# wafgo/rt-depth-map

Hardware: AMD Instinct MI355X
Metric: stereo-pairs/sec, 1280x720 d=64 9x9 SAD (higher is better)
Workload: dtype u8

## Files before the change

rt-depth-map_amd/csrc/k_search_ring.hip:

```cpp
#include "rtdm_select.h"
#include "rtdm_border.h"
#include "rtdm_border2.h"
#include "rtdm_search.h"

#include <cmath>
#include <cstdlib>
#include <type_traits>
#include <utility>

namespace rtdm {

struct RingGeom {
    int x0, nx;
    int rs;
    uint32_t lastmask;
    int tiles, strips;
    unsigned nitems;
    unsigned chunk;
    uint32_t rdelta;
    int rebase;
    unsigned nborder;
    int bgx, bgy;
    int b2;
};

__host__ __device__ constexpr int ring_rpg(int D, int LPP) { return D >= 96 ? 4 : LPP; }

template <int D, int WS, int LPP = 2>
struct RingCfg {
    static constexpr int RPG = ring_rpg(D, LPP);
    static constexpr bool SPLIT = LPP != 2 || D >= 48 || (D == 32 && (WS == 9 || WS == 5));
    static constexpr bool B64 = SPLIT && D == 64;
    using Rec = SelRecord<D, B64>;
    static constexpr int NP = (WS + 3) / 4;
    static constexpr int W1 = WS + 1;
    static constexpr int PPW = 64 / LPP;
    static constexpr bool PAIR = D == 64 && WS == 9 && LPP == 4;
    static constexpr int LPG = PAIR ? 2 * LPP : LPP;
    static constexpr int GPW = 64 / LPG;
    static constexpr int DL = D / LPG;
    static constexpr int NGL = DL / 4;
    static constexpr int NRL = DL / 2;
    static constexpr int NL = PAIR ? NP + 1 : NP;
    static constexpr int NW = NGL + NL - 1;
    static constexpr int LWD = GPW + NP;
    static constexpr int RWD = GPW + D / 4 + NP;
    static constexpr int ITEMS = (LWD + RWD + 63) / 64;
    static constexpr int SLOT = ITEMS * 64;
    static constexpr int TRIP = (W1 % RPG == 0) ? W1 : (2 * W1 % RPG == 0) ? 2 * W1 : 4 * W1;
    static_assert(W1 % 2 == 0 && TRIP % RPG == 0 && TRIP % W1 == 0, "block sizes are odd");
    static constexpr bool STATIC_SLOTS = ITEMS == 1 && TRIP % 4 == 0;
    static constexpr int NSLOT = STATIC_SLOTS ? 4 : 3;
    static constexpr int TEXD = (PAIR ? (TRIP + RPG) : (W1 + RPG)) * PPW / 2;
    static constexpr int STG = (NSLOT * SLOT + TEXD + 3) & ~3;
    static constexpr int PREC = D / 2 + D / 16;
    static constexpr int PREC_PAIR = LPG * PREC;
    __host__ __device__ static constexpr int pair_rec(int p, int o) { return p * PREC_PAIR + o * PREC + 2 * (p & 1) + 8 * (p >> 1); }
    static constexpr int REC_DWORDS = PAIR ? pair_rec(GPW - 1, LPG - 1) + PREC + 2 : PPW * RPG * Rec::DWORDS;
    static constexpr int WAVE_LDS = STG + REC_DWORDS;
    static constexpr int RING_REGS = W1 * NRL * (PAIR ? 2 : 1);
    static constexpr int W3_LIMIT = 112;
    static constexpr int WAVES = PAIR ? 3 : LPP >= 8 ? 2 : LPP == 4 ? (RING_REGS <= 80 ? 4 : (RING_REGS <= 96 && NRL <= 8) ? 3 : 2) : (RING_REGS <= 72 && NRL <= 8) ? 4 : RING_REGS <= W3_LIMIT ? 3 : 2;
    static constexpr int TILE = 4 * PPW;
    static constexpr bool FUSE_BORDER = WAVES < 4 && !PAIR;
    static constexpr bool FUSE_BORDER2 = D <= 192;
    static constexpr bool ROW_PTRS = !(LPP == 2 && RING_REGS > 88 && WAVES == 3);
};

template <int D, int WS, int LPP, bool BORDER>
struct RingBounds {
    using C = RingCfg<D, WS, LPP>;
    static constexpr int WAVES = BORDER && C::WAVES > 1 && !C::PAIR ? C::WAVES - 1 : C::WAVES;
};

template <int D, int WS, int LPP = 2>
struct RingState {
    uint64_t P[RingCfg<D, WS, LPP>::W1][RingCfg<D, WS, LPP>::NGL];
    uint64_t P2[RingCfg<D, WS, LPP>::PAIR ? RingCfg<D, WS, LPP>::W1 : 1][RingCfg<D, WS, LPP>::NGL];
};

template <int D, int WS, int LPP = 2>
struct RowRegs { uint64_t win[RingCfg<D, WS, LPP>::NW]; uint32_t l[RingCfg<D, WS, LPP>::NL]; };

typedef __attribute__((address_space(3))) const uint32_t* lds_cptr;
__device__ __forceinline__ uint32_t lds_addr(const uint32_t* q) { return (uint32_t)(uintptr_t)(lds_cptr)q; }
__device__ __forceinline__ lds_cptr lds_at(uint32_t a) { return (lds_cptr)(uintptr_t)a; }

template <int D, int WS, int LPP, typename PTR>
__device__ __forceinline__ void ring_load_row(PTR lp, PTR rp, PTR rpo, RowRegs<D, WS, LPP>& rw)
{
    using C = RingCfg<D, WS, LPP>;
#pragma unroll
    for (int k = 0; k < C::NL; ++k) rw.l[k] = lp[k];
#pragma unroll
    for (int j = 0; j < C::NW; ++j) {
        const PTR wp = (j & 1) ? rpo + (j - 1) : rp + j;
        rw.win[j] = (uint64_t)wp[0] | ((uint64_t)wp[1] << 32);
    }
}

template <int D, int WS, int LPP, int K, int NRLc>
__device__ __forceinline__ void ring_step(RingState<D, WS, LPP>& st, const RowRegs<D, WS, LPP>& rw, uint32_t lastmask, uint32_t capb,
                                          uint32_t& tnew, uint32_t (&S)[NRLc])
{
    using C = RingCfg<D, WS, LPP>;
    auto& P = st.P;
    constexpr int NP = C::NP, NGL = C::NGL, W1 = C::W1;
    constexpr int KP = (K + W1 - 1) % W1, KO = (K + 1) % W1;
    uint32_t l[NP];
#pragma unroll
    for (int k = 0; k < NP; ++k) l[k] = rw.l[k];
    l[NP - 1] &= lastmask;
#pragma unroll
    for (int k = 0; k < NP - 1; ++k) tnew = __builtin_amdgcn_sad_u8(l[k], capb, tnew);
    tnew = __builtin_amdgcn_msad_u8(capb, l[NP - 1], tnew);
#pragma unroll
    for (int j = 0; j < C::NW; ++j) {
#pragma unroll
        for (int k = 0; k < NP; ++k) {
            const int gi = j - k;
            if (gi >= 0 && gi < NGL) {
                const uint64_t acc = k == 0 ? P[KP][gi] : P[K][gi];
                if (k == NP - 1) P[K][gi] = __builtin_amdgcn_mqsad_pk_u16_u8(rw.win[j], l[k], acc);
                else             P[K][gi] = __builtin_amdgcn_qsad_pk_u16_u8(rw.win[j], l[k], acc);
            }
        }
    }
#pragma unroll
    for (int gi = 0; gi < NGL; ++gi) {
        S[2 * gi] = (uint32_t)P[K][gi] - (uint32_t)P[KO][gi];
        S[2 * gi + 1] = (uint32_t)(P[K][gi] >> 32) - (uint32_t)(P[KO][gi] >> 32);
    }
}

__device__ __forceinline__ uint64_t ring_add_halves(uint64_t a, uint64_t b)
{
    typedef uint32_t u2 __attribute__((ext_vector_type(2)));
    return __builtin_bit_cast(uint64_t, __builtin_bit_cast(u2, a) + __builtin_bit_cast(u2, b));
}

template <int D, int WS, int LPP, int K, int NRLc>
__device__ __forceinline__ void ring_step_pair(RingState<D, WS, LPP>& st, const RowRegs<D, WS, LPP>& rw, uint32_t (&S)[NRLc], uint32_t (&S2)[NRLc])
{
    using C = RingCfg<D, WS, LPP>;
    static_assert(C::PAIR && WS % 4 == 1, "the two windows share whole dwords only for w = 1 (mod 4)");
    constexpr int NP = C::NP, NGL = C::NGL, W1 = C::W1;
    constexpr int KP = (K + W1 - 1) % W1, KO = (K + 1) % W1;
    const uint32_t lf = rw.l[0] & 0xff000000u, ll = rw.l[NP] & 0x000000ffu;
    uint64_t sh[NGL], e1[NGL], e2[NGL];
#pragma unroll
    for (int j = 0; j < C::NW; ++j) {
#pragma unroll
        for (int k = 0; k <= NP; ++k) {
            const int gi = j - k;
            if (gi >= 0 && gi < NGL) {
                if (k == 0)       e1[gi] = __builtin_amdgcn_mqsad_pk_u16_u8(rw.win[j], lf, st.P[KP][gi]);
                else if (k == NP) e2[gi] = __builtin_amdgcn_mqsad_pk_u16_u8(rw.win[j], ll, st.P2[KP][gi]);
                else              sh[gi] = __builtin_amdgcn_qsad_pk_u16_u8(rw.win[j], rw.l[k], k == 1 ? (uint64_t)0 : sh[gi]);
            }
        }
    }
#pragma unroll
    for (int gi = 0; gi < NGL; ++gi) {
        st.P[K][gi] = ring_add_halves(e1[gi], sh[gi]);
        st.P2[K][gi] = ring_add_halves(e2[gi], sh[gi]);
        S[2 * gi] = (uint32_t)st.P[K][gi] - (uint32_t)st.P[KO][gi];
        S[2 * gi + 1] = (uint32_t)(st.P[K][gi] >> 32) - (uint32_t)(st.P[KO][gi] >> 32);
        S2[2 * gi] = (uint32_t)st.P2[K][gi] - (uint32_t)st.P2[KO][gi];
        S2[2 * gi + 1] = (uint32_t)(st.P2[K][gi] >> 32) - (uint32_t)(st.P2[KO][gi] >> 32);
    }
}

template <int N>
__device__ __forceinline__ void pin(uint32_t (&v)[N])
{
#pragma unroll
    for (int i = 0; i < N; ++i) asm volatile("" : "+v"(v[i]));
}

template <typename T>
__device__ __forceinline__ __attribute__((address_space(3))) T* lds_as(uint32_t a) { return (__attribute__((address_space(3))) T*)(uintptr_t)a; }

template <typename C>
struct RingTexture {
    static constexpr int TRIP = C::TRIP, RPG = C::RPG, WS = C::W1 - 1;
    static_assert(RPG == 4 && TRIP % RPG == 0 && TRIP >= WS + RPG && (WS - 1) % RPG == 0, "one straddling group, at U = w - 1");
    static constexpr int RING_BYTES = C::PPW * TRIP * 2;
    uint32_t a_row, a_edge;
    uint32_t a_term, a_col;
    uint32_t a_ring, a_wrap;
    uint32_t w_lo, w_hi;
    uint32_t carry;

    __device__ __forceinline__ void init(uint32_t stg_addr, uint32_t tex_addr, int p, int h)
    {
        const int k = h >> 1, j = h & 1, colw = 2 * p + j;
        a_row = stg_addr + (uint32_t)(k * C::SLOT + p + 1) * 4;
        a_edge = stg_addr + (uint32_t)(k * C::SLOT + p) * 4 + (j ? 12u : 3u);
        a_col = tex_addr + RING_BYTES + (uint32_t)colw * (RPG * 2);
        a_term = a_col + 2 * k;
        a_ring = tex_addr + (uint32_t)(colw * TRIP + k) * 2;
        a_wrap = tex_addr + (uint32_t)(colw * TRIP + (k + TRIP - 1) % TRIP) * 2;
        w_lo = k >= 1 ? 0x00010001u : 0x00000001u;
        w_hi = k >= 3 ? 0x00010001u : k == 2 ? 0x00000001u : 0u;
        carry = 0;
        asm volatile("" : "+v"(a_row), "+v"(a_edge), "+v"(a_term), "+v"(a_col), "+v"(a_ring), "+v"(a_wrap), "+v"(w_lo), "+v"(w_hi));
    }
    template <int U>
    __device__ __forceinline__ uint32_t back() const
    {
        constexpr int lo = U - WS;
        if constexpr (lo < 0 && lo + RPG - 1 >= 0) {
            static_assert(lo == -1, "a_wrap is the address for U = w - 1");
            return *lds_as<const uint16_t>(a_wrap);
        } else {
            constexpr int idx = (lo + TRIP) % TRIP;
            static_assert(idx + RPG - 1 < TRIP, "no wrap inside the group");
            return *lds_as<const uint16_t>(a_ring + idx * 2);
        }
    }
    __device__ __forceinline__ void term(uint32_t capb) const
    {
        const uint32_t l1 = *lds_as<const uint32_t>(a_row), l2 = *lds_as<const uint32_t>(a_row + 4);
        const uint32_t e = *lds_as<const uint8_t>(a_edge);
        uint32_t t = __builtin_amdgcn_sad_u8(l1, capb, 0u);
        t = __builtin_amdgcn_sad_u8(l2, capb, t);
        t = __builtin_amdgcn_msad_u8(capb, e, t);
        *lds_as<uint16_t>(a_term) = (uint16_t)t;
    }
    template <int U>
    __device__ __forceinline__ uint32_t prefix()
    {
        const uint64_t q = *lds_as<const uint64_t>(a_col);
        const sel_us2 lo = __builtin_bit_cast(sel_us2, (uint32_t)q), hi = __builtin_bit_cast(sel_us2, (uint32_t)(q >> 32));
        const sel_us2 ones = __builtin_bit_cast(sel_us2, 0x00010001u);
        uint32_t own = __builtin_amdgcn_udot2(lo, __builtin_bit_cast(sel_us2, w_lo), carry, false);
        own = __builtin_amdgcn_udot2(hi, __builtin_bit_cast(sel_us2, w_hi), own, false);
        carry = __builtin_amdgcn_udot2(lo, ones, carry, false);
        carry = __builtin_amdgcn_udot2(hi, ones, carry, false);
        *lds_as<uint16_t>(a_ring + U * 2) = (uint16_t)own;
        return own;
    }
};

template <typename F, int... U>
__device__ __forceinline__ void ring_for_groups(std::integer_sequence<int, U...>, F&& f)
{ (void)(f(std::integral_constant<int, U>{}) && ...); }
template <typename F, int... R>
__device__ __forceinline__ void ring_for_rows(std::integer_sequence<int, R...>, F&& f)
{ (f(std::integral_constant<int, R>{}), ...); }

template <int D, int WS, int LPP, bool FUSE>
__global__ __launch_bounds__(256, (RingBounds<D, WS, LPP, FUSE>::WAVES)) void k_search_ring(Plane8 Lp, Plane8 Rp, Plane16W disp, uint16_t* cost, BMGeom g, RingGeom rg,
                                                                                   BorderGeom bg, Border2Geom b2g)
{
    using C = RingCfg<D, WS, LPP>;
    constexpr int NGL = C::NGL, NRL = C::NRL, W1 = C::W1, LWD = C::LWD, SLOT = C::SLOT, ITEMS = C::ITEMS, PPW = C::PPW, RPG = C::RPG;
    constexpr int GPW = C::GPW;
    constexpr bool SPLIT = C::SPLIT, PAIR = C::PAIR;
    static_assert(!PAIR || (SPLIT && C::STATIC_SLOTS && C::LPG == 2 * RPG), "the paired layout: one owner lane per (column, row) of a group");
    constexpr int RECD = C::Rec::DWORDS;
    extern __shared__ __attribute__((aligned(16))) uint32_t lds[];

    unsigned fi = blockIdx.x;
    if constexpr (FUSE) {
        if (fi < rg.nborder) {
            const unsigned per = (unsigned)(rg.bgx * rg.bgy), fr = fi / per, id = fi - fr * per;
            if (C::FUSE_BORDER2 && rg.b2) {
                const int wave = __builtin_amdgcn_readfirstlane((int)(threadIdx.x >> 6));
                border2_body<D, C::NP>(Lp, Rp, disp, cost, g, b2g, (int)(id % rg.bgx) * 4 + wave, (int)(id / rg.bgx), (int)fr);
            } else if constexpr (C::FUSE_BORDER) {
                border_body<(D + 63) / 64>((unsigned char*)lds, Lp, Rp, disp, cost, g, bg, (int)(id % rg.bgx), (int)(id / rg.bgx), (int)fr);
            }
            return;
        }
        fi -= rg.nborder;
    }
    if (rg.chunk) fi = (fi & 7u) * rg.chunk + (fi >> 3);
    if (fi >= rg.nitems) return;
    const int b_tile = (int)(fi % rg.tiles), b_strip = (int)((fi / rg.tiles) % rg.strips), f = (int)(fi / (rg.tiles * rg.strips));

    const int tid = threadIdx.x, lane = tid & 63;
    const int phi = __builtin_amdgcn_readfirstlane(tid >> 6);
    const int p = lane & (GPW - 1), h = lane / GPW;
    const int x_tile = rg.x0 + b_tile * C::TILE;
    const int xw = PAIR ? x_tile + (phi >> 1) * (C::TILE / 2) + 2 * (phi & 1) : x_tile + phi;
    const int hrow = PAIR ? h >> 1 : h;
    const int x = xw + 4 * p + (PAIR ? h & 1 : 0);
    const bool active = x < rg.x0 + rg.nx;
    const int ys0 = g.vy0 + b_strip * rg.rs;
    const int ys1 = min(ys0 + rg.rs, g.vy1);
    if (ys0 >= ys1) return;
    const int r = g.r;
    const uint8_t* Lb = Lp.base + (size_t)f * Lp.frame;
    constexpr int PAIR_SHIFT = PAIR ? 3 : 0;
    const int Lbase = g.lofs + xw - r;
    const int Rbase = g.rofs + xw - r;
    const uint32_t capb = (uint32_t)(g.cap + PREFILTER_BIAS) * 0x01010101u;

    uint32_t* stg = lds + phi * C::WAVE_LDS;
    unsigned short* ptr = (unsigned short*)(stg + C::NSLOT * SLOT);
    unsigned short* ptw = ptr + W1 * PPW;
    const bool owner = PAIR || RPG == LPP || h < RPG;
    const unsigned short* ptw_own = ptw + (owner ? hrow : 0) * PPW + p;
    struct None {};
    [[maybe_unused]] std::conditional_t<PAIR, RingTexture<C>, None> tex;
    static_assert(!PAIR || ((C::NSLOT * SLOT) % 2 == 0 && C::WAVE_LDS % 2 == 0), "the row terms of a column are read as 8 bytes");
    uint32_t* scr = stg + C::STG + (PAIR ? C::pair_rec(p, h) : (owner ? lane : 0) * RECD);
    uint32_t* const rec0 = stg + C::STG + (PAIR ? C::pair_rec(p, 0) : p * RECD);
    uint32_t* scr_w = rec0 + h * NRL;
    using GSel = GroupSelectRec<D, C::LPG, C::B64>;
    unsigned short* scr_m = (unsigned short*)(rec0 + D / 2) + h * (NRL / 4);
    if constexpr (SPLIT) GSel::init(scr);

    const int row0 = ys0 - r;
    const int Hm1 = g.H - 1;
    const uint8_t* rowp = Lb + (size_t)row0 * Lp.pitch - PAIR_SHIFT;
    uint32_t loff[ITEMS];
#pragma unroll
    for (int it = 0; it < ITEMS; ++it) {
        const int idx = lane + it * 64;
        const bool isr = idx >= LWD;
        const int m = isr ? (PAIR ? min(idx - LWD, C::RWD - 1) : idx - LWD) : idx;
        loff[it] = (uint32_t)((isr ? Rbase : Lbase) + 4 * m) + (isr ? rg.rdelta : 0u);
    }
    int next_row = row0;
    uint32_t pre[2][ITEMS];
    auto issue = [&](auto Sc) {
        constexpr int SET = decltype(Sc)::value;
#pragma unroll
        for (int it = 0; it < ITEMS; ++it) {
            asm volatile("" : "+v"(loff[it]));
            pre[SET][it] = *(const uint32_t*)(rowp + loff[it]);
        }
        rowp += next_row < Hm1 ? Lp.pitch : 0;
        ++next_row;
    };
    auto commit = [&](auto Sc, auto slot) {
        constexpr int SET = decltype(Sc)::value;
#pragma unroll
        for (int it = 0; it < ITEMS; ++it) stg[slot * SLOT + lane + it * 64] = pre[SET][it];
        __builtin_amdgcn_wave_barrier();
    };
    using Set0 = std::integral_constant<int, 0>;
    using Set1 = std::integral_constant<int, 1>;

    RingState<D, WS, LPP> st;
#pragma unroll
    for (int k = 0; k < W1; ++k)
#pragma unroll
        for (int i = 0; i < NGL; ++i) {
            st.P[k][i] = 0;
            if constexpr (PAIR) st.P2[k][i] = 0;
        }
    if constexpr (PAIR) {
        constexpr int RINGD = RingTexture<C>::RING_BYTES / 4;
#pragma unroll
        for (int i = 0; i < (RINGD + 63) / 64; ++i)
            if (i * 64 + 63 < RINGD || lane + i * 64 < RINGD) stg[C::NSLOT * SLOT + lane + i * 64] = 0;
        tex.init(lds_addr(stg), lds_addr(stg + C::NSLOT * SLOT), p, h);
    } else {
#pragma unroll
        for (int k = 0; k < W1; ++k) ptr[k * PPW + p] = 0;
    }
    uint32_t pt = 0;

    const int nsteps = (ys1 - ys0) + WS - 1;
    const int nstepsg = (nsteps + RPG - 1) / RPG * RPG;
    issue(Set0{}); issue(Set1{});
    commit(Set0{}, 0); commit(Set1{}, 1);
    issue(Set0{});

    char* const db = (char*)(disp.base + (size_t)f * disp.frame_e);
    char* const cb = (char*)(cost + (size_t)f * g.H * g.Ws);
    const int col = g.lofs + x;
    constexpr int TF = (WS - 1) / RPG * RPG;
    uint32_t dofs = (uint32_t)(((long long)(ys0 + TF + hrow - (WS - 1)) * (long long)disp.pitch_e + col) * 2);
    uint32_t cofs = (uint32_t)(((long long)(ys0 + TF + hrow - (WS - 1)) * (long long)g.Ws + col) * 2);
    const uint32_t dstep = (uint32_t)(disp.pitch_e * 2 * RPG), cstep = (uint32_t)(g.Ws * 2 * RPG);
    const bool masked_col = g.mask_cols && (col < g.vx0 || col >= g.vx1);

    uint32_t S[RPG][NRL];
    int sl_cur = 0;
    uint32_t la_cur = lds_addr(stg + p), ra_cur = lds_addr(stg + LWD + p + h * NGL), ro_cur = ra_cur + 4;
    if constexpr (C::STATIC_SLOTS) asm volatile("" : "+v"(la_cur), "+v"(ra_cur), "+v"(ro_cur));
    const auto lds_row = [&](auto SLc, RowRegs<D, WS, LPP>& rw) {
        if constexpr (C::STATIC_SLOTS) {
            constexpr uint32_t off = (uint32_t)(decltype(SLc)::value * SLOT * 4);
            ring_load_row<D, WS, LPP>(lds_at(la_cur + off), lds_at(ra_cur + off), lds_at(ro_cur + off), rw);
        } else if constexpr (C::ROW_PTRS) {
            asm volatile("" : "+v"(la_cur), "+v"(ra_cur), "+v"(ro_cur));
            ring_load_row<D, WS, LPP>(lds_at(la_cur), lds_at(ra_cur), lds_at(ro_cur), rw);
            const uint32_t adv = (uint32_t)((sl_cur == 2 ? -2 * SLOT : SLOT) * 4);
            la_cur += adv; ra_cur += adv; ro_cur += adv;
        } else {
            int li = sl_cur * SLOT + p, ri = sl_cur * SLOT + LWD + p + h * NGL, one = 1;
            asm volatile("" : "+v"(li), "+v"(ri), "+v"(one));
            ring_load_row<D, WS, LPP, const uint32_t*>(stg + li, stg + ri, stg + ri + one, rw);
        }
    };
    [[maybe_unused]] uint32_t tback = 0, tpre = 0;
    auto step = [&](auto Kc, auto SLc, auto Rc, auto Uc, const RowRegs<D, WS, LPP>& rw, uint32_t (&Sr)[NRL], uint32_t (&Sr2)[NRL]) {
        constexpr int K = decltype(Kc)::value;
        using SetIn = std::integral_constant<int, (K + 1) & 1>;
        using SetOut = std::integral_constant<int, K & 1>;
        issue(SetIn{});
        uint32_t tnew = 0;
        constexpr int KO = (K + 1) % W1;
        if constexpr (PAIR) {
            constexpr int R = decltype(Rc)::value, U = decltype(Uc)::value;
            if constexpr (R == 2) { tback = tex.template back<U>(); tex.term(capb); }
            if constexpr (R == 3) tpre = tex.template prefix<U>();
            ring_step_pair<D, WS, LPP, K>(st, rw, Sr, Sr2);
            pin(Sr2);
        } else {
            ring_step<D, WS, LPP, K>(st, rw, rg.lastmask, capb, tnew, Sr);
            pt += tnew;
            const uint32_t told = ptr[KO * PPW + p];
            ptr[K * PPW + p] = (unsigned short)pt;
            ptw[decltype(Rc)::value * PPW + p] = (unsigned short)(pt - told);
        }
        pin(Sr);
        if constexpr (C::STATIC_SLOTS) {
            commit(SetOut{}, std::integral_constant<int, (decltype(SLc)::value + 2) % 4>{});
        } else {
            const int sl_new = sl_cur == 0 ? 2 : sl_cur - 1;
            sl_cur = sl_cur == 2 ? 0 : sl_cur + 1;
            commit(SetOut{}, sl_new);
        }
    };

    int trips_since_rebase = 0;
    for (int t0 = 0; t0 < nstepsg; t0 += C::TRIP) {
        if (rg.rebase && ++trips_since_rebase > rg.rebase) {
            trips_since_rebase = 1;
#pragma unroll
            for (int i = 0; i < NGL; ++i) {
                const uint32_t blo = (uint32_t)st.P[1][i], bhi = (uint32_t)(st.P[1][i] >> 32);
#pragma unroll
                for (int k = 1; k < W1; ++k) {
                    const uint32_t lo = (uint32_t)st.P[k][i] - blo, hi = (uint32_t)(st.P[k][i] >> 32) - bhi;
                    st.P[k][i] = (uint64_t)lo | ((uint64_t)hi << 32);
                }
                if constexpr (PAIR) {
                    const uint32_t blo2 = (uint32_t)st.P2[1][i], bhi2 = (uint32_t)(st.P2[1][i] >> 32);
#pragma unroll
                    for (int k = 1; k < W1; ++k) {
                        const uint32_t lo = (uint32_t)st.P2[k][i] - blo2, hi = (uint32_t)(st.P2[k][i] >> 32) - bhi2;
                        st.P2[k][i] = (uint64_t)lo | ((uint64_t)hi << 32);
                    }
                }
            }
        }
        ring_for_groups(std::make_integer_sequence<int, C::TRIP / RPG>{}, [&](auto Uc) -> bool {
            constexpr int U = RPG * decltype(Uc)::value;
            const int t = t0 + U;
            if (t >= nstepsg) return false;
            GSel gsel;
            ring_for_rows(std::make_integer_sequence<int, RPG>{}, [&](auto Rc) {
                constexpr int R = decltype(Rc)::value;
                RowRegs<D, WS, LPP> rw;
                using SL = std::integral_constant<int, (U + R) % 4>;
                lds_row(SL{}, rw);
                uint32_t S2[NRL] = {};
                step(std::integral_constant<int, (U + R) % W1>{}, SL{}, Rc, std::integral_constant<int, U>{}, rw, S[R], S2);
                if constexpr (PAIR) {
                    gsel.template row<R>(S[R], scr_w + 2 * R * C::PREC, scr_m + 2 * R * (C::PREC * 2));
                    gsel.template row<R>(S2, scr_w + (2 * R + 1) * C::PREC, scr_m + (2 * R + 1) * (C::PREC * 2));
                } else if constexpr (SPLIT) gsel.template row<R>(S[R], scr_w + R * (PPW * RECD), scr_m + R * (PPW * RECD * 2));
            });
            if (t + RPG - 1 < WS - 1) return true;
            const int y = ys0 + (t - (WS - 1)) + hrow;
            const bool row_ok = owner && y >= ys0 && y < ys1;
            const uint32_t dof = dofs, cof = cofs;
            dofs += dstep; cofs += cstep;
            int tsum;
            if constexpr (PAIR) tsum = (int)((tpre - tback) & 0xffffu);
            else tsum = *ptw_own;
            const bool dead = !active | !row_ok | masked_col | (tsum < g.tex);
            if (__builtin_amdgcn_ballot_w64(!dead) == 0) {
                if (active && row_ok) *(int16_t*)(db + dof) = (int16_t)g.filtered;
            } else {
                int m1; bool fail;
                int out;
                if constexpr (SPLIT) {
                    int uq = g.uniq;
                    asm volatile("" : "+s"(uq));
                    out = gsel.finish(tsum, g, uq > 0, scr, &m1, &fail);
                } else {
                    uint32_t rr[D / 2];
#pragma unroll
                    for (int i = 0; i < NRL; ++i) {
                        const auto sw = __builtin_amdgcn_permlane32_swap(S[0][i], S[RPG - 1][i], false, false);
                        rr[i] = sw[0]; rr[NRL + i] = sw[1];
                    }
                    out = select_disparity_lds<D>(rr, tsum, g, scr, &m1, &fail);
                }
                if (active && row_ok) {
                    if (!fail && g.want_cost) *(uint16_t*)(cb + cof) = (uint16_t)m1;
                    *(int16_t*)(db + dof) = (int16_t)(masked_col ? g.filtered : out);
                }
            }
            return true;
        });
    }
}


static int ring_rows_cap(const BMGeom& g) { return 65535 / (g.w * 2 * g.cap) - g.w - 6; }
static int ring_rebase_trips(const BMGeom& g, int lpp)
{
    const int W1 = g.w + 1, rpg = ring_rpg(g.D, lpp);
    const int trip = (W1 % rpg == 0) ? W1 : (2 * W1 % rpg == 0) ? 2 * W1 : 4 * W1;
    return ring_rows_cap(g) / trip;
}
static int ring_min_strips(const BMGeom& g, int lpp, int nrows)
{ return ring_rebase_trips(g, lpp) > 0 ? 1 : max(1, (nrows + ring_rows_cap(g) - 1) / ring_rows_cap(g)); }

#ifdef RTDM_RING_DEV
#define RTDM_RING_TABLE(X) RTDM_RING_DEV
#else
#define RTDM_RING_TABLE(X) X(64, 9, 2) X(64, 7, 2) X(64, 5, 2) X(32, 7, 2) X(32, 9, 2) X(32, 11, 2) X(32, 13, 2) X(48, 7, 2) X(48, 9, 2) \
                           X(16, 5, 2) X(16, 7, 2) X(16, 9, 2) X(64, 9, 4) X(64, 7, 4) X(64, 5, 4) X(64, 11, 4) X(64, 13, 4) \
                           X(128, 7, 8) X(128, 9, 8) X(128, 11, 8) X(128, 13, 8) X(96, 7, 4) X(96, 9, 4) X(96, 11, 4) X(96, 13, 4) X(48, 11, 2) X(48, 13, 2) \
                           X(16, 11, 2) X(16, 13, 2) X(32, 5, 2) X(32, 15, 2) X(48, 5, 2) X(64, 15, 4) X(128, 15, 8) \
                           X(192, 9, 8) X(192, 11, 8) X(192, 13, 8) X(192, 15, 8) X(256, 9, 16) X(256, 11, 16) X(256, 13, 16) X(256, 15, 16)
#endif

static std::atomic<int> g_ring_switch{0};
void ring_set_mode(int mode)
{
    const int m = mode < 0 ? -1 : mode == 0 ? 0 : 1, lpp = (mode == 2 || mode == 4 || mode == 8) ? mode : 0;
    g_ring_switch.store((m + 1) | (lpp << 8), std::memory_order_relaxed);
}
static int ring_mode() { return (g_ring_switch.load(std::memory_order_relaxed) & 0xff) - 1; }
static int ring_forced_lpp() { return g_ring_switch.load(std::memory_order_relaxed) >> 8; }

static int ring_lpp(const BMGeom& g)
{
    int have = 0;
#define X(DD, WW, LL) if (g.D == DD && g.w == WW) have |= LL;
    RTDM_RING_TABLE(X)
#undef X
    const int want = ring_forced_lpp();
    if (want && (have & want) == want) return want;
    return (have & 16) ? 16 : (have & 8) ? 8 : (have & 4) ? 4 : (have & 2) ? 2 : 0;
}

static RingForm ring_form_of(const BMGeom& g, int lpp)
{
#define X(DD, WW, LL) if (g.D == DD && g.w == WW && lpp == LL) { using C = RingCfg<DD, WW, LL>; return RingForm{LL, C::WAVES, C::FUSE_BORDER2, C::FUSE_BORDER, C::TILE}; }
    RTDM_RING_TABLE(X)
#undef X
    return RingForm{};
}

RingForm ring_form(const BMGeom& g)
{
    const RingForm none{};
    if (ring_mode() == 0) return none;
    if (2L * g.cap * g.w * g.w > 32766) return none;
    if (2L * g.cap * g.w * g.w >= 0x7C00) return none;
    if (ring_rows_cap(g) < 2) return none;
    if ((size_t)g.H * (size_t)g.Ws * 2 >= ((size_t)1 << 32)) return none;
    return ring_form_of(g, ring_lpp(g));
}

int ring_strips_model(const SearchPlan& plan, const BMGeom& g, int n)
{
    const int tile = 256 / plan.lanes, tiles = (plan.nx + tile - 1) / tile, nrows = g.vy1 - g.vy0;
    const int slots = 256 * ring_form_of(g, plan.lanes).waves;
    const int smin = ring_min_strips(g, plan.lanes, nrows), smax = max(smin, (nrows + 15) / 16);
    const float fill = 0.5f * (float)(g.w - 1);
    int s = (int)(sqrtf((float)nrows * (float)slots / (fill * (float)tiles * (float)n)) + 0.5f);
    s = max(smin, min(s, smax));
    if ((long)tiles * s * n < 6L * slots) {
        float best = 1e30f;
        for (int c = smin; c <= smax; ++c) {
            const int rs = (nrows + c - 1) / c, ce = (nrows + rs - 1) / rs;
            const long rounds = ((long)tiles * ce * n + slots - 1) / slots;
            const float t = (float)rounds * ((float)rs + fill + 2.0f);
            if (t < best) { best = t; s = ce; }
        }
    }
    return s;
}

template <int D, int WS, int LPP>
static void ring_launch_one(const SearchPlan& plan, Plane8 Lp, Plane8 Rp, Plane16W disp, void* cost, const BMGeom& g, int n, hipStream_t stream,
                            int strips_hint)
{
    using C = RingCfg<D, WS, LPP>;
    RingGeom rg;
    rg.rdelta = (uint32_t)(Rp.base - Lp.base);
    rg.x0 = plan.x0; rg.nx = plan.nx;
    const int rem = g.w - 4 * (C::NP - 1);
    rg.lastmask = rem >= 4 ? 0xffffffffu : ((1u << (8 * rem)) - 1u);
    const int nrows = g.vy1 - g.vy0;
    const int tiles = (rg.nx + C::TILE - 1) / C::TILE;
    int strips = strips_hint > 0 ? strips_hint : ring_strips_model(plan, g, n);
    strips = max(strips, ring_min_strips(g, LPP, nrows));
    rg.rebase = ring_rebase_trips(g, LPP);
    strips = max(1, min(strips, nrows));
    rg.rs = (nrows + strips - 1) / strips;
    strips = (nrows + rg.rs - 1) / rg.rs;
    rg.tiles = tiles; rg.strips = strips;
    rg.nitems = (unsigned)tiles * strips * n;
    rg.chunk = (rg.nitems + 7) / 8;
    const unsigned grid = rg.chunk * 8;
    BorderGeom bg{};
    Border2Geom b2g{};
    size_t blds = 0;
    rg.nborder = 0; rg.bgx = rg.bgy = 0; rg.b2 = 0;
    if (plan.place == BorderPlace::FUSED && plan.border.form != BorderForm::NONE) {
        const BorderPlan& b = plan.border;
        if (b.form == BorderForm::ROWS) { b2g = b.rows; rg.b2 = 1; }
        else { bg = b.disp; blds = b.lds; }
        rg.bgx = b.gx; rg.bgy = b.gy;
        rg.nborder = (unsigned)(rg.bgx * rg.bgy) * (unsigned)n;
    }
    const size_t ldsb = max((size_t)4 * C::WAVE_LDS * sizeof(uint32_t), blds);
    const auto launch = [&](auto Fc) {
        constexpr bool F = decltype(Fc)::value;
        constexpr size_t ring_lds = (size_t)4 * C::WAVE_LDS * sizeof(uint32_t);
        const size_t most = C::FUSE_BORDER ? max(ring_lds, border_lds_bytes(D, WS)) : ring_lds;
        static OncePerDevice once;
        if (most > 48 * 1024 && once.first()) {
            int dev = 0, lds_max = 0;
            size_t want = max(most, (size_t)64 * 1024);
            if (hipGetDevice(&dev) == hipSuccess &&
                hipDeviceGetAttribute(&lds_max, hipDeviceAttributeMaxSharedMemoryPerMultiprocessor, dev) == hipSuccess && lds_max > 0)
                want = min(want, (size_t)lds_max);
            (void)hipGetLastError();
            (void)hipFuncSetAttribute((const void*)k_search_ring<D, WS, LPP, F>, hipFuncAttributeMaxDynamicSharedMemorySize, (int)want);
        }
        hipLaunchKernelGGL((k_search_ring<D, WS, LPP, F>), dim3(grid + rg.nborder), dim3(256), ldsb, stream, Lp, Rp, disp, (uint16_t*)cost, g, rg, bg, b2g);
    };
    if (rg.nborder) launch(std::true_type{});
    else launch(std::false_type{});
}

void launch_search_ring(const SearchPlan& plan, Plane8 Lp, Plane8 Rp, Plane16W disp, void* cost, const BMGeom& g, int n, hipStream_t stream,
                        int strips)
{
#define X(DD, WW, LL) if (g.D == DD && g.w == WW && plan.lanes == LL) { ring_launch_one<DD, WW, LL>(plan, Lp, Rp, disp, cost, g, n, stream, strips); return; }
    RTDM_RING_TABLE(X)
#undef X
}

}
```

Baseline: 77670.

## Prefetch next LDS row and deepen global load queue in paired ring kernel

For the paired configuration, the next row's LDS window is loaded into double-buffered registers while the current row's SAD step runs. Global row loads are queued four deep instead of two, so each load has more steps to land before its commit. Texture term and prefix LDS reads are split from their arithmetic so they can issue early. This hides LDS and global latency at the cost of more live registers, which could reduce occupancy or cause spills.

```diff
diff --git a/rt-depth-map_amd/csrc/k_search_ring.hip b/rt-depth-map_amd/csrc/k_search_ring.hip
--- a/rt-depth-map_amd/csrc/k_search_ring.hip
+++ b/rt-depth-map_amd/csrc/k_search_ring.hip
@@ -65,6 +65,9 @@
     static constexpr bool FUSE_BORDER = WAVES < 4 && !PAIR;
     static constexpr bool FUSE_BORDER2 = D <= 192;
     static constexpr bool ROW_PTRS = !(LPP == 2 && RING_REGS > 88 && WAVES == 3);
+    static constexpr bool PREFETCH = PAIR;
+    static constexpr int LOAD_SETS = PREFETCH ? 4 : 2;
+    static_assert(!PREFETCH || (STATIC_SLOTS && NSLOT == 4), "the slot of row t + 1 is a constant of the step, distinct from that of row t + 2");
 };
 
 template <int D, int WS, int LPP, bool BORDER>
@@ -219,19 +222,21 @@
             return *lds_as<const uint16_t>(a_ring + idx * 2);
         }
     }
-    __device__ __forceinline__ void term(uint32_t capb) const
+    struct TermIn { uint32_t l1, l2, e; };
+    __device__ __forceinline__ TermIn term_load() const
+    { return TermIn{*lds_as<const uint32_t>(a_row), *lds_as<const uint32_t>(a_row + 4), *lds_as<const uint8_t>(a_edge)}; }
+    __device__ __forceinline__ void term(uint32_t capb, const TermIn& in) const
     {
-        const uint32_t l1 = *lds_as<const uint32_t>(a_row), l2 = *lds_as<const uint32_t>(a_row + 4);
-        const uint32_t e = *lds_as<const uint8_t>(a_edge);
+        const uint32_t l1 = in.l1, l2 = in.l2, e = in.e;
         uint32_t t = __builtin_amdgcn_sad_u8(l1, capb, 0u);
         t = __builtin_amdgcn_sad_u8(l2, capb, t);
         t = __builtin_amdgcn_msad_u8(capb, e, t);
         *lds_as<uint16_t>(a_term) = (uint16_t)t;
     }
+    __device__ __forceinline__ uint64_t prefix_load() const { return *lds_as<const uint64_t>(a_col); }
     template <int U>
-    __device__ __forceinline__ uint32_t prefix()
+    __device__ __forceinline__ uint32_t prefix(uint64_t q)
     {
-        const uint64_t q = *lds_as<const uint64_t>(a_col);
         const sel_us2 lo = __builtin_bit_cast(sel_us2, (uint32_t)q), hi = __builtin_bit_cast(sel_us2, (uint32_t)(q >> 32));
         const sel_us2 ones = __builtin_bit_cast(sel_us2, 0x00010001u);
         uint32_t own = __builtin_amdgcn_udot2(lo, __builtin_bit_cast(sel_us2, w_lo), carry, false);
@@ -325,7 +330,9 @@
         loff[it] = (uint32_t)((isr ? Rbase : Lbase) + 4 * m) + (isr ? rg.rdelta : 0u);
     }
     int next_row = row0;
-    uint32_t pre[2][ITEMS];
+    constexpr int NPRE = C::LOAD_SETS;
+    constexpr bool QUEUED = NPRE > 2;
+    uint32_t pre[NPRE][ITEMS];
     auto issue = [&](auto Sc) {
         constexpr int SET = decltype(Sc)::value;
 #pragma unroll
@@ -370,6 +377,8 @@
     issue(Set0{}); issue(Set1{});
     commit(Set0{}, 0); commit(Set1{}, 1);
     issue(Set0{});
+    if constexpr (QUEUED)
+        ring_for_rows(std::make_integer_sequence<int, NPRE - 2>{}, [&](auto Kc) { issue(std::integral_constant<int, decltype(Kc)::value + 1>{}); });
 
     char* const db = (char*)(disp.base + (size_t)f * disp.frame_e);
     char* const cb = (char*)(cost + (size_t)f * g.H * g.Ws);
@@ -400,20 +409,28 @@
         }
     };
     [[maybe_unused]] uint32_t tback = 0, tpre = 0;
-    auto step = [&](auto Kc, auto SLc, auto Rc, auto Uc, const RowRegs<D, WS, LPP>& rw, uint32_t (&Sr)[NRL], uint32_t (&Sr2)[NRL]) {
+    auto step = [&](auto Kc, auto SLc, auto Rc, auto Uc, auto&& ahead, const RowRegs<D, WS, LPP>& rw, uint32_t (&Sr)[NRL], uint32_t (&Sr2)[NRL]) {
         constexpr int K = decltype(Kc)::value;
         using SetIn = std::integral_constant<int, (K + 1) & 1>;
         using SetOut = std::integral_constant<int, K & 1>;
-        issue(SetIn{});
+        if constexpr (QUEUED) issue(std::integral_constant<int, NPRE - 1>{});
+        else issue(SetIn{});
         uint32_t tnew = 0;
         constexpr int KO = (K + 1) % W1;
         if constexpr (PAIR) {
             constexpr int R = decltype(Rc)::value, U = decltype(Uc)::value;
-            if constexpr (R == 2) { tback = tex.template back<U>(); tex.term(capb); }
-            if constexpr (R == 3) tpre = tex.template prefix<U>();
+            [[maybe_unused]] typename RingTexture<C>::TermIn tin;
+            [[maybe_unused]] uint64_t tq;
+            if constexpr (R == 2) { tback = tex.template back<U>(); tin = tex.term_load(); }
+            if constexpr (R == 3) tq = tex.prefix_load();
+            ahead();
+            if constexpr (C::PREFETCH) __builtin_amdgcn_sched_barrier(0x214);
             ring_step_pair<D, WS, LPP, K>(st, rw, Sr, Sr2);
             pin(Sr2);
+            if constexpr (R == 2) { asm volatile("" : "+v"(tin.l1), "+v"(tin.l2), "+v"(tin.e)); tex.term(capb, tin); }
+            if constexpr (R == 3) { asm volatile("" : "+v"(tq)); tpre = tex.template prefix<U>(tq); }
         } else {
+            ahead();
             ring_step<D, WS, LPP, K>(st, rw, rg.lastmask, capb, tnew, Sr);
             pt += tnew;
             const uint32_t told = ptr[KO * PPW + p];
@@ -421,7 +438,14 @@
             ptw[decltype(Rc)::value * PPW + p] = (unsigned short)(pt - told);
         }
         pin(Sr);
-        if constexpr (C::STATIC_SLOTS) {
+        if constexpr (QUEUED) {
+            static_assert(C::STATIC_SLOTS, "the queued loads go with static slots");
+            commit(Set0{}, std::integral_constant<int, (decltype(SLc)::value + 2) % 4>{});
+#pragma unroll
+            for (int it = 0; it < ITEMS; ++it)
+#pragma unroll
+                for (int k = 0; k + 1 < NPRE; ++k) pre[k][it] = pre[k + 1][it];
+        } else if constexpr (C::STATIC_SLOTS) {
             commit(SetOut{}, std::integral_constant<int, (decltype(SLc)::value + 2) % 4>{});
         } else {
             const int sl_new = sl_cur == 0 ? 2 : sl_cur - 1;
@@ -430,6 +454,8 @@
         }
     };
 
+    [[maybe_unused]] RowRegs<D, WS, LPP> rwp[2];
+    if constexpr (C::PREFETCH) lds_row(std::integral_constant<int, 0>{}, rwp[0]);
     int trips_since_rebase = 0;
     for (int t0 = 0; t0 < nstepsg; t0 += C::TRIP) {
         if (rg.rebase && ++trips_since_rebase > rg.rebase) {
@@ -459,11 +485,17 @@
             GSel gsel;
             ring_for_rows(std::make_integer_sequence<int, RPG>{}, [&](auto Rc) {
                 constexpr int R = decltype(Rc)::value;
-                RowRegs<D, WS, LPP> rw;
                 using SL = std::integral_constant<int, (U + R) % 4>;
-                lds_row(SL{}, rw);
                 uint32_t S2[NRL] = {};
-                step(std::integral_constant<int, (U + R) % W1>{}, SL{}, Rc, std::integral_constant<int, U>{}, rw, S[R], S2);
+                if constexpr (C::PREFETCH) {
+                    pin(rwp[(U + R) & 1].l);
+                    const auto ahead = [&] { lds_row(std::integral_constant<int, (U + R + 1) % 4>{}, rwp[(U + R + 1) & 1]); };
+                    step(std::integral_constant<int, (U + R) % W1>{}, SL{}, Rc, std::integral_constant<int, U>{}, ahead, rwp[(U + R) & 1], S[R], S2);
+                } else {
+                    RowRegs<D, WS, LPP> rw;
+                    lds_row(SL{}, rw);
+                    step(std::integral_constant<int, (U + R) % W1>{}, SL{}, Rc, std::integral_constant<int, U>{}, [] {}, rw, S[R], S2);
+                }
                 if constexpr (PAIR) {
                     gsel.template row<R>(S[R], scr_w + 2 * R * C::PREC, scr_m + 2 * R * (C::PREC * 2));
                     gsel.template row<R>(S2, scr_w + (2 * R + 1) * C::PREC, scr_m + (2 * R + 1) * (C::PREC * 2));
```

After: 79280 (median of 6 runs). +2.1%, better.
